# ViacheslavTimofeev/tpu_superresolution

Hardware: AMD Instinct MI355X
Metric: HR pixels/sec, SwinIR x4 train step, 64x64 LR, bs=32/GPU (higher is better)
Workload: dtype bf16; 1 GPU; BASELINE cfg3: SwinIR classical x4 (dim 180, 6x6 blocks, window 8) train step = fwd + L1 + bwd + clip 1.0 + AdamW, 64x64 LR patches -> 256x256 HR, random-init weights, drop_path 0.1; every step starts from the seeded weights and fresh AdamW state; batch_per_gpu=32, global_batch=32, parallelism=dp1

## Files before the change

### tpu_superresolution_amd/csrc/api.hip

```cpp
#include <stdarg.h>
#include <stdio.h>
#include <string.h>

#include "adamw.h"
#include "kernels.h"
#include "wgrad.h"

static thread_local char g_err[512] = "";

SrkOptTls& srk_opt_tls() {
  static thread_local SrkOptTls t = {};
  return t;
}

static SrkOpt** opt_table() {
  static SrkOpt* table[SRK_NUM_OPTS] = {};
  return table;
}

void srk_opt_register(SrkOpt* o) {
  if (o->id >= 0 && o->id < SRK_NUM_OPTS) opt_table()[o->id] = o;
}

void srk_opt_scope_begin(SrkOptTls* saved) {
// ... 308 lines not shown
  srk_gemm_stream_tune_get(&v[0], &v[1], &v[2], &v[3]);
  return v[which];
}
int tune_set(int which, int value) {
  int v[4];
  srk_gemm_stream_tune_get(&v[0], &v[1], &v[2], &v[3]);
  v[which] = value;
  srk_gemm_stream_tune(v[0], v[1], v[2], v[3]);
  return SRK_OK;
}
int wtune_get(int which) {
  int rows, nt;
  srk_wgrad_stream_tune_get(&rows, &nt);
  return which == 0 ? rows : nt;
}

struct OptEntry {
  const char* name;
  int (*get)();
  int (*set)(int);
};

const OptEntry kOptions[] = {
    {"gemm_stream", [] { return srk_gemm_stream_enabled(); }, [](int v) { srk_gemm_stream_enable(v); return (int)SRK_OK; }},
    {"attn_bwd_fused", [] { return srk_attn_bwd_fused_enabled(); }, [](int v) { srk_attn_bwd_fused_enable(v); return (int)SRK_OK; }},
    {"attn_fused", [] { return srk_attn_fused_mode(); }, [](int v) { srk_attn_fused_enable(v); return (int)SRK_OK; }},
    {"wgrad_stream_w8", [] { return srk_wgrad_w8_enabled(); }, [](int v) { srk_wgrad_w8_enable(v); return (int)SRK_OK; }},
    {"block_light", [] { return srk_block_light_enabled(); }, [](int v) { srk_block_light_enable(v); return (int)SRK_OK; }},
    {"mlp_bwd_fused", [] { return srk_mlp_bwd_fused_enabled(); }, [](int v) { srk_mlp_bwd_fused_enable(v); return (int)SRK_OK; }},
    {"mlp_dgelu_store", [] { return srk_mlp_dgelu_store_enabled(); }, [](int v) { srk_mlp_dgelu_store_enable(v); return (int)SRK_OK; }},
    {"mlp_fused", [] { return srk_mlp_fused_enabled(); }, [](int v) { srk_mlp_fused_enable(v); return (int)SRK_OK; }},
    {"wgrad_stream", [] { return srk_wgrad_stream_enabled(); }, [](int v) { srk_wgrad_stream_enable(v); return (int)SRK_OK; }},
    {"conv_wgrad_taps", [] { return srk_conv_wgrad_taps_mode(); }, [](int v) { srk_conv_wgrad_taps_enable(v); return (int)SRK_OK; }},
    {"wgrad_partials", [] { return srk_wgrad_partials_enabled(); }, [](int v) { srk_wgrad_partials_enable(v); return (int)SRK_OK; }},
    {"wgrad_stream_rows", [] { return wtune_get(0); },
     [](int v) {
       SRK_REQUIRE(v == 32 || v == 64, SRK_E_SHAPE, "wgrad_stream_rows: 32/64");
       srk_wgrad_stream_tune(v, -1);
       return (int)SRK_OK;
     }},
    {"wgrad_stream_nt", [] { return wtune_get(1); }, [](int v) { srk_wgrad_stream_tune(0, v != 0); return (int)SRK_OK; }},
    {"gemm_stream_bm", [] { return tune_get(0); },
     [](int v) {
       SRK_REQUIRE(v == 0 || v == 16 || v == 32 || v == 64, SRK_E_SHAPE, "gemm_stream_bm: 0/16/32/64");
       return tune_set(0, v);
     }},
    {"gemm_stream_ks2", [] { return tune_get(1); }, [](int v) { return tune_set(1, v < 0 ? -1 : (v != 0)); }},
    {"gemm_stream_split", [] { return tune_get(2); }, [](int v) { return tune_set(2, v < 0 ? -1 : (v != 0)); }},
    {"gemm_stream_nb", [] { return tune_get(3); },
     [](int v) {
       SRK_REQUIRE(v == 0 || v == 4 || v == 8, SRK_E_SHAPE, "gemm_stream_nb: 0/4/8");
       return tune_set(3, v);
     }},
    {"probe_stride", [] { return g_probe.stride; },
     [](int v) {
       SRK_REQUIRE(v >= 1 && v <= 1024, SRK_E_SHAPE, "probe_stride: 1..1024");
       g_probe.stride = v;
       return (int)SRK_OK;
     }},
};

const OptEntry* find_option(const char* name) {
  for (const OptEntry& e : kOptions)
    if (strcmp(name, e.name) == 0) return &e;
  return nullptr;
}
// ... 158 lines not shown
```

### tpu_superresolution_amd/csrc/common.h

```cpp
#pragma once
#include <hip/hip_runtime.h>
#include <stdint.h>

#include "../../include/srk.h"

typedef unsigned short bf16_t;
typedef __attribute__((ext_vector_type(8))) short bf16x8_t;
typedef __attribute__((ext_vector_type(4))) short bf16x4_t;
typedef __attribute__((ext_vector_type(4))) float f32x4_t;

#define SRK_WAVE 64

void srk_set_error(const char* fmt, ...);
int srk_check_launch(const char* what);

constexpr int SRK_MAX_DEVICES = 64;
int srk_current_device();
int srk_device_cus();
enum SrkOptId {
  OPT_MLP_FUSED, OPT_MLP_BWD_FUSED, OPT_GEMM_STREAM, OPT_TUNE_BM, OPT_TUNE_KS2, OPT_TUNE_SPLIT, OPT_TUNE_NB, OPT_ATTN_BWD_FUSED,
  OPT_ATTN_FUSED, OPT_BLOCK_LIGHT, OPT_TAPS_ENABLED, OPT_TAPS_DMA, OPT_WGRAD_STREAM, OPT_WGRAD_ROWS, OPT_WGRAD_NT, OPT_WGRAD_W8,
  OPT_WGRAD_PARTIALS, OPT_MLP_DGELU_STORE, SRK_NUM_OPTS
};
struct SrkOptTls {
  int v[SRK_NUM_OPTS];
  unsigned on;
};
SrkOptTls& srk_opt_tls();
struct SrkOpt;
void srk_opt_register(SrkOpt* o);
void srk_opt_scope_begin(SrkOptTls* saved);
void srk_opt_scope_end(const SrkOptTls& saved);
struct SrkOpt {
  int id;
  int value;
  SrkOpt(int id_, int v) : id(id_), value(v) { srk_opt_register(this); }
  operator int() const {
    const SrkOptTls& t = srk_opt_tls();
    return ((t.on >> id) & 1u) ? t.v[id] : value;
  }
  SrkOpt& operator=(int v) {
    SrkOptTls& t = srk_opt_tls();
    if ((t.on >> id) & 1u) t.v[id] = v;
    else value = v;
    return *this;
  }
  SrkOpt(const SrkOpt&) = delete;
  SrkOpt& operator=(const SrkOpt&) = delete;
};

template <class T>
struct SrkPerDevice {
  T v[SRK_MAX_DEVICES] = {};
  T& here() { return v[srk_current_device()]; }
};
// ... 214 lines not shown
```

### tpu_superresolution_amd/csrc/convwgrad.hip

```cpp
#include "wgrad.h"

#ifndef SRK_NT_TAPS
#define SRK_NT_TAPS 0
#endif

namespace {

constexpr int CT = 64;
constexpr int SP = 64 + 16;
constexpr int HALO = CT + 2;
constexpr int XROWS = 3 * HALO;
constexpr int YPIECES = CT * 8 / 256;
constexpr int XPIECES = (XROWS * 8 + 255) / 256;

template <bool SHUF>
__global__ __launch_bounds__(256) void conv_wgrad_taps_kernel(const WgradParams p, int ntiles, int chunks_per) {
  extern __shared__ __attribute__((aligned(16))) unsigned char smem[];
  bf16_t* Ys = reinterpret_cast<bf16_t*>(smem);
  bf16_t* Xs = Ys + 2 * CT * SP;

  const int tid = threadIdx.x, lane = tid & 63;
  const int wave = __builtin_amdgcn_readfirstlane(tid >> 6);
  const int r16 = lane & 15, g = lane >> 4;
  const int logical = xcd_remap(blockIdx.x, gridDim.x);
  const int bsplit = logical / ntiles, btile = logical - bsplit * ntiles;
  const int ntn = p.N / 64;
  const int tn = btile % ntn, tk = btile / ntn;
  const int n0 = tn * 64, k0 = tk * 64;
  const int c_begin = bsplit * chunks_per;
  const int c_end = min(p.M / CT, c_begin + chunks_per);
  if (c_begin >= c_end) return;
  const int hw = p.H * p.W;
// ... 120 lines not shown
      srk_set_error("conv wgrad: cannot reserve %zu bytes of LDS", lds);
      return SRK_E_LAUNCH;
    }
    configured = true;
  }
  const int tiles = (p.N / 64) * (p.K / 64);
  const int nchunks = p.M / CT;
  int splits = 256 / tiles;
  if (splits < 1) splits = 1;
  if (splits > nchunks) splits = nchunks;
  const int chunks_per = cdiv(nchunks, splits);
  splits = cdiv(nchunks, chunks_per);
  srk_probe_pre(FAM_WGRAD_CONV, stream, p.flops, p.bytes);
  hipLaunchKernelGGL((conv_wgrad_taps_kernel<SHUF>), dim3(tiles * splits), dim3(256), lds, stream, p, tiles, chunks_per);
  srk_probe_post(FAM_WGRAD_CONV, stream);
  return srk_check_launch("conv wgrad (all taps)");
}

__device__ uint4 g_zero_page[8];

constexpr int TD_YROWS = CT, TD_STAGE_ROWS = CT + XROWS;
constexpr int TD_STAGE_BYTES = TD_STAGE_ROWS * 128;
constexpr int TD_RING = 4;
constexpr int TD_PIECES = TD_STAGE_ROWS * 8;
constexpr int TD_PPW = TD_PIECES / 4;
constexpr int TD_NI = (TD_PPW + 63) / 64;

__device__ __forceinline__ const bf16_t* tr_addr_swz64(const bf16_t* tile, int rbase, int c0, int lane) {
  const int ll = lane & 15;
  const int row = rbase + (ll >> 2);
  return tile + row * 64 + (((c0 >> 4) ^ ((row >> 1) & 3)) << 4) + ((ll & 3) << 2);
}

template <bool SHUF>
__global__ __launch_bounds__(256) void conv_wgrad_taps_dma_kernel(const WgradParams p, int ntiles, int chunks_per, float* partial,
                                                                  int nsplit) {
  extern __shared__ __attribute__((aligned(16))) unsigned char smem[];
  const unsigned ring_base = (unsigned)(size_t)smem;
  const int tid = threadIdx.x, lane = tid & 63;
  const int wave = __builtin_amdgcn_readfirstlane(tid >> 6);
  const int r16 = lane & 15, g = lane >> 4;
  const int logical = xcd_remap(blockIdx.x, gridDim.x);
  const int bsplit = logical / ntiles, btile = logical - bsplit * ntiles;
  const int ntn = p.N / 64;
  const int tn = btile % ntn, tk = btile / ntn;
  const int n0 = tn * 64, k0 = tk * 64;
  const int c_begin = bsplit * chunks_per;
  const int c_end = min(p.M / CT, c_begin + chunks_per);
  if (c_begin >= c_end) return;
  const int hw = p.H * p.W;
  const bf16_t* zero = reinterpret_cast<const bf16_t*>(g_zero_page);

  int loff[TD_NI];
  int lrp[TD_NI];
#pragma unroll
  for (int i = 0; i < TD_NI; ++i) {
    const int qq = wave * TD_PPW + i * 64 + lane;
    const int row = qq >> 3, pos = qq & 7;
    const int c = (((pos >> 1) ^ ((row >> 1) & 3)) << 1) | (pos & 1);
    if (row < TD_YROWS) {
      lrp[i] = -1;
      if constexpr (SHUF) {
        const int nn = n0 + c * 8;
        const int ij = nn / p.Cs, cc = nn - ij * p.Cs;
        const int si = ij / p.r, sj = ij - si * p.r;
        loff[i] = (si * (p.W * p.r) + row * p.r + sj) * p.Cs + cc;
      } else {
        loff[i] = row * p.ldy + n0 + c * 8;
      }
    } else {
// ... 42 lines not shown
    if (it + TD_RING - 2 < nrun) srk_wait_vmcnt<TD_NI*(TD_RING - 2)>(); else srk_wait_vmcnt<0>();
    srk_lds_barrier();
    if (it + TD_RING - 1 < nrun) issue(c_begin + it + TD_RING - 1);
    const bf16_t* ys = reinterpret_cast<const bf16_t*>(smem + (it % TD_RING) * TD_STAGE_BYTES);
    const bf16_t* xs = ys + TD_YROWS * 64;
#pragma unroll
    for (int ks = 0; ks < 2; ++ks) {
      bf16x8_t yf[4];
#pragma unroll
      for (int i = 0; i < 4; ++i) {
        const bf16x4_t lo = lds_tr_read(tr_addr_swz64(ys, 32 * ks + 4 * g, 16 * i, lane));
        const bf16x4_t hi = lds_tr_read(tr_addr_swz64(ys, 32 * ks + 16 + 4 * g, 16 * i, lane));
        yf[i] = bf16x8_t{lo[0], lo[1], lo[2], lo[3], hi[0], hi[1], hi[2], hi[3]};
      }
#pragma unroll
      for (int q = 0; q < 9; ++q) {
        const int cg = 9 * wave + q;
        const int tap = cg >> 2;
        const int xb = (tap / 3) * HALO + (tap % 3);
        const bf16x4_t lo = lds_tr_read(tr_addr_swz64(ys, TD_YROWS + xb + 32 * ks + 4 * g, 16 * (cg & 3), lane));
        const bf16x4_t hi = lds_tr_read(tr_addr_swz64(ys, TD_YROWS + xb + 32 * ks + 16 + 4 * g, 16 * (cg & 3), lane));
        const bf16x8_t xf = bf16x8_t{lo[0], lo[1], lo[2], lo[3], hi[0], hi[1], hi[2], hi[3]};
#pragma unroll
        for (int i = 0; i < 4; ++i) acc[i][q] = __builtin_amdgcn_mfma_f32_16x16x32_bf16(yf[i], xf, acc[i][q], 0, 0, 0);
      }
      if (do_bias) {
#pragma unroll
        for (int i = 0; i < 4; ++i) accb[i] = __builtin_amdgcn_mfma_f32_16x16x32_bf16(yf[i], ones, accb[i], 0, 0, 0);
      }
    }
    (void)xs;
  }

  if (partial != nullptr) {
    f32x4_t* slab = reinterpret_cast<f32x4_t*>(partial) + ((size_t)btile * nsplit + bsplit) * WS_SLAB_VEC + (size_t)wave * 36 * 64 + lane;
#pragma unroll
    for (int i = 0; i < 4; ++i)
#pragma unroll
      for (int q = 0; q < 9; ++q) slab[(i * 9 + q) * 64] = acc[i][q];
  }
#pragma unroll
  for (int i = 0; i < 4; ++i) {
    const int n = n0 + 16 * i + 4 * g;
    if (partial == nullptr) {
#pragma unroll
      for (int q = 0; q < 9; ++q) {
        const int cg = 9 * wave + q;
        const long long col = (long long)(cg >> 2) * p.K + k0 + 16 * (cg & 3) + r16;
#pragma unroll
        for (int e = 0; e < 4; ++e) atomicAdd(p.dW + (long long)(n + e) * p.ldw + col, acc[i][q][e]);
      }
    }
    if (do_bias && r16 == 0) {
#pragma unroll
      for (int e = 0; e < 4; ++e) atomicAdd(p.db + n + e, accb[i][e]);
    }
  }
}

__global__ __launch_bounds__(256) void conv_wgrad_taps_reduce_kernel(const WgradParams p, const float* __restrict__ partial, int nsplit) {
  const int btile = blockIdx.x / 36;
  const int v = (blockIdx.x - btile * 36) * 256 + threadIdx.x;
  const int ntn = p.N / 64;
  const int tn = btile % ntn, tk = btile / ntn;
  const f32x4_t* src = reinterpret_cast<const f32x4_t*>(partial) + (size_t)btile * nsplit * WS_SLAB_VEC + v;
  f32x4_t sum = f32x4_t{0.f, 0.f, 0.f, 0.f};
  int s = 0;
  for (; s + 8 <= nsplit; s += 8) {
    f32x4_t t[8];
#pragma unroll
    for (int u = 0; u < 8; ++u) t[u] = src[(size_t)(s + u) * WS_SLAB_VEC];
#pragma unroll
    for (int u = 0; u < 8; ++u) sum += t[u];
  }
  for (; s < nsplit; ++s) sum += src[(size_t)s * WS_SLAB_VEC];
  const int lane = v & 63, t = v >> 6;
  const int q = t % 9, i = (t / 9) % 4, wave = t / 36;
  const int r16 = lane & 15, g = lane >> 4;
  const int n = tn * 64 + 16 * i + 4 * g;
  const int cg = 9 * wave + q;
  const long long col = (long long)(cg >> 2) * p.K + tk * 64 + 16 * (cg & 3) + r16;
#pragma unroll
  for (int e = 0; e < 4; ++e) atomicAdd(p.dW + (long long)(n + e) * p.ldw + col, sum[e]);
}

SrkOpt g_taps_dma{OPT_TAPS_DMA, 1};

template <bool SHUF>
int launch_taps_dma(const WgradParams& p, hipStream_t stream) {
  constexpr int lds = TD_RING * TD_STAGE_BYTES;
  static SrkPerDevice<bool> configured_pd; bool& configured = configured_pd.here();
  if (!configured) {
    if (hipFuncSetAttribute(reinterpret_cast<const void*>(&conv_wgrad_taps_dma_kernel<SHUF>), hipFuncAttributeMaxDynamicSharedMemorySize,
                            lds) != hipSuccess) {
      srk_set_error("conv wgrad (dma): cannot reserve %d bytes of LDS", lds);
      return SRK_E_LAUNCH;
    }
    configured = true;
  }
  const int tiles = (p.N / 64) * (p.K / 64);
  const int nchunks = p.M / CT;
  int splits = 256 / tiles;
  if (splits < 1) splits = 1;
  if (splits > nchunks) splits = nchunks;
  const int chunks_per = cdiv(nchunks, splits);
  splits = cdiv(nchunks, chunks_per);
  float* partial =
      srk_wgrad_partials_enabled() && splits > 1 ? srk_wgrad_scratch(stream, (size_t)tiles * splits * WS_SLAB_VEC * 16) : nullptr;
  srk_probe_pre(FAM_WGRAD_CONV, stream, p.flops, p.bytes);
  hipLaunchKernelGGL((conv_wgrad_taps_dma_kernel<SHUF>), dim3(tiles * splits), dim3(256), lds, stream, p, tiles, chunks_per, partial,
                     splits);
  if (partial) hipLaunchKernelGGL(conv_wgrad_taps_reduce_kernel, dim3(tiles * 36), dim3(256), 0, stream, p, partial, splits);
  srk_probe_post(FAM_WGRAD_CONV, stream);
  return srk_check_launch("conv wgrad (all taps, dma)");
}

template <int COP>
__global__ __launch_bounds__(256) void smallconv_wgrad_mfma_kernel(const bf16_t* __restrict__ x, const float* __restrict__ gy,
                                                                   float* __restrict__ dW, float* __restrict__ db, int B, int H, int W,
                                                                   int Cin, int CinP, int Co, int ntiles, int chunks_per) {
  extern __shared__ __attribute__((aligned(16))) unsigned char smem[];
  bf16_t* Yh = reinterpret_cast<bf16_t*>(smem);
  bf16_t* Yl = Yh + 2 * CT * 16;
  bf16_t* Xs = Yl + 2 * CT * 16;
  const int tid = threadIdx.x, lane = tid & 63;
  const int wave = __builtin_amdgcn_readfirstlane(tid >> 6);
  const int r16 = lane & 15, g = lane >> 4;
  const int logical = xcd_remap(blockIdx.x, gridDim.x);
  const int bsplit = logical / ntiles, tk = logical - bsplit * ntiles;
  const int k0 = tk * 64;
  const int M = B * H * W;
  const int c_begin = bsplit * chunks_per;
  const int c_end = min(M / CT, c_begin + chunks_per);
  if (c_begin >= c_end) return;
  const int hw = H * W;
  for (int i = tid; i < 2 * 2 * CT * 16 / 2; i += 256) reinterpret_cast<unsigned*>(Yh)[i] = 0u;

  constexpr int YP = CT * COP / 4;
  float4 ry = make_float4(0.f, 0.f, 0.f, 0.f);
  uint4 rx[XPIECES];
  const int nxb = W / CT;
  auto load_stage = [&](int ch) {
    const int b = ch / (H * nxb), r = ch - b * (H * nxb);
    const int xb = r / H, y = r - xb * H, x0 = xb * CT;
    const int m0 = b * hw + y * W + x0;
    if (tid < YP) ry = *reinterpret_cast<const float4*>(gy + (long long)m0 * COP + tid * 4);
#pragma unroll
    for (int t = 0; t < XPIECES; ++t) {
      const int pid = tid + 256 * t;
      const int hr = pid >> 3, c8 = pid & 7;
      const int rr = hr / HALO, px = hr - rr * HALO;
// ... 62 lines not shown
        const bf16x8_t xf = bf16x8_t{lo[0], lo[1], lo[2], lo[3], hi[0], hi[1], hi[2], hi[3]};
        acc[q] = __builtin_amdgcn_mfma_f32_16x16x32_bf16(yfh, xf, acc[q], 0, 0, 0);
        acc[q] = __builtin_amdgcn_mfma_f32_16x16x32_bf16(yfl, xf, acc[q], 0, 0, 0);
      }
      if (do_bias) {
        accb = __builtin_amdgcn_mfma_f32_16x16x32_bf16(yfh, ones, accb, 0, 0, 0);
        accb = __builtin_amdgcn_mfma_f32_16x16x32_bf16(yfl, ones, accb, 0, 0, 0);
      }
    }
    if (ch + 1 < c_end) store_stage(buf ^ 1);
    __syncthreads();
  }

#pragma unroll
  for (int q = 0; q < 9; ++q) {
    const int cg = 9 * wave + q;
    const int tap = cg >> 2, k = k0 + 16 * (cg & 3) + r16;
#pragma unroll
    for (int e = 0; e < 4; ++e) {
      const int n = 4 * g + e;
      if (n < Co && k < Cin) atomicAdd(dW + ((long long)(n * Cin) + k) * 9 + tap, acc[q][e]);
    }
  }
  if (do_bias && r16 == 0) {
#pragma unroll
    for (int e = 0; e < 4; ++e)
      if (4 * g + e < Co) atomicAdd(db + 4 * g + e, accb[e]);
  }
}

template <int COP>
int launch_smallconv_mfma(const bf16_t* x, const float* gy, float* dW, float* db, int B, int H, int W, int Cin, int CinP, int Co,
                          hipStream_t stream) {
  constexpr size_t lds = (size_t)(2 * 2 * CT * 16 + 2 * XROWS * SP) * sizeof(bf16_t);
  static SrkPerDevice<bool> configured_pd; bool& configured = configured_pd.here();
  if (!configured) {
    if (hipFuncSetAttribute(reinterpret_cast<const void*>(&smallconv_wgrad_mfma_kernel<COP>), hipFuncAttributeMaxDynamicSharedMemorySize,
                            (int)lds) != hipSuccess) {
      srk_set_error("smallconv wgrad: cannot reserve %zu bytes of LDS", lds);
      return SRK_E_LAUNCH;
    }
    configured = true;
  }
  const int tiles = CinP / 64;
  const int nchunks = (B * H * W) / CT;
  int splits = 512 / tiles;
  if (splits > nchunks) splits = nchunks;
  const int chunks_per = cdiv(nchunks, splits);
  splits = cdiv(nchunks, chunks_per);
  hipLaunchKernelGGL((smallconv_wgrad_mfma_kernel<COP>), dim3(tiles * splits), dim3(256), lds, stream, x, gy, dW, db, B, H, W, Cin, CinP, Co,
                     tiles, chunks_per);
  return srk_check_launch("smallconv wgrad (mfma)");
}

__device__ __forceinline__ void split_bf16x8(const float (&v)[8], bf16x8_t& hi, bf16x8_t& lo) {
#pragma unroll
  for (int i = 0; i < 8; ++i) {
    const bf16_t h = f2bf(v[i]);
    hi[i] = (short)h;
    lo[i] = (short)f2bf(v[i] - bf2f(h));
  }
}

__global__ __launch_bounds__(256) void imghead_dgrad_mfma_kernel(const float* __restrict__ gy, const float* __restrict__ wgt,
                                                                 bf16_t* __restrict__ dx, int B, int H, int W, int Cin, int Co, int nchunks) {
  constexpr int TP = 64 + 8;
  __shared__ __attribute__((aligned(16))) bf16_t T[64 * TP];
  const int tid = threadIdx.x, lane = tid & 63;
  const int wave = __builtin_amdgcn_readfirstlane(tid >> 6);
  const int r16 = lane & 15, g = lane >> 4;

  bf16x8_t wh[4][2], wl[4][2];
#pragma unroll
  for (int j = 0; j < 4; ++j)
#pragma unroll
    for (int ks = 0; ks < 2; ++ks) {
      float v[8];
#pragma unroll
      for (int jj = 0; jj < 8; ++jj) {
        const int k = 32 * ks + 8 * g + jj;
        const int tap = k >> 2, co = k & 3, ci = 16 * j + r16;
        v[jj] = (tap < 9 && co < Co && ci < Cin) ? wgt[((co * Cin) + ci) * 9 + tap] : 0.f;
      }
      split_bf16x8(v, wh[j][ks], wl[j][ks]);
    }

  const int hw = H * W;
  for (int c = blockIdx.x; c < nchunks; c += gridDim.x) {
    const int pix = c * 64 + 16 * wave + r16;
    const int b = pix / hw, rem = pix - b * hw;
    const int y = rem / W, x = rem - y * W;
    f32x4_t acc[4];
#pragma unroll
    for (int j = 0; j < 4; ++j) acc[j] = f32x4_t{0.f, 0.f, 0.f, 0.f};
// ... 11 lines not shown
        }
        v[4 * half] = gv.x; v[4 * half + 1] = gv.y; v[4 * half + 2] = gv.z; v[4 * half + 3] = gv.w;
      }
      bf16x8_t xh, xl;
      split_bf16x8(v, xh, xl);
#pragma unroll
      for (int j = 0; j < 4; ++j) {
        acc[j] = __builtin_amdgcn_mfma_f32_16x16x32_bf16(wh[j][ks], xh, acc[j], 0, 0, 0);
        acc[j] = __builtin_amdgcn_mfma_f32_16x16x32_bf16(wl[j][ks], xh, acc[j], 0, 0, 0);
        acc[j] = __builtin_amdgcn_mfma_f32_16x16x32_bf16(wh[j][ks], xl, acc[j], 0, 0, 0);
      }
    }
#pragma unroll
    for (int j = 0; j < 4; ++j)
      *reinterpret_cast<uint2*>(T + (16 * wave + r16) * TP + 16 * j + 4 * g) = pack_bf4(acc[j][0], acc[j][1], acc[j][2], acc[j][3]);
    srk_lds_barrier();
#pragma unroll
    for (int t = 0; t < 2; ++t) {
      const int pid = tid + 256 * t;
      const int row = pid >> 3, c8 = pid & 7;
      *reinterpret_cast<uint4*>(dx + ((long long)c * 64 + row) * 64 + c8 * 8) = *reinterpret_cast<const uint4*>(T + row * TP + c8 * 8);
    }
    srk_lds_barrier();
  }
}

}

void srk_conv_wgrad_taps_enable(int on) {
  g_taps_enabled = on ? 1 : 0;
  g_taps_dma = on >= 2 ? 1 : 0;
}
int srk_conv_wgrad_taps_mode() { return g_taps_enabled ? (g_taps_dma ? 2 : 1) : 0; }

int srk_launch_conv_wgrad_taps(const WgradParams& p, hipStream_t stream) {
  if (!g_taps_enabled || !p.conv || p.W % CT != 0 || p.N % 64 != 0 || p.K % 64 != 0 || p.ldx % 8 != 0) return SRK_WGRAD_NOT_COVERED;
  if (p.r > 1) {
    if (p.Cs % 8 != 0 || p.N != p.r * p.r * p.Cs) return SRK_WGRAD_NOT_COVERED;
    return g_taps_dma ? launch_taps_dma<true>(p, stream) : launch_taps<true>(p, stream);
  }
  if (p.ldy % 8 != 0) return SRK_WGRAD_NOT_COVERED;
  return g_taps_dma ? launch_taps_dma<false>(p, stream) : launch_taps<false>(p, stream);
}

int srk_launch_smallconv_wgrad_mfma(const bf16_t* x, const float* gy, float* dW, float* db, int B, int H, int W, int Cin, int CinP,
                                    int Co, int CoP, hipStream_t stream) {
  if (!g_taps_enabled || W % CT != 0 || CinP % 64 != 0 || Co > CoP || ((long long)B * H * W) % CT != 0) return SRK_WGRAD_NOT_COVERED;
  if (CoP == 4) return launch_smallconv_mfma<4>(x, gy, dW, db, B, H, W, Cin, CinP, Co, stream);
  if (CoP == 16) return launch_smallconv_mfma<16>(x, gy, dW, db, B, H, W, Cin, CinP, Co, stream);
  return SRK_WGRAD_NOT_COVERED;
}

int srk_launch_imghead_dgrad_mfma(const float* gy, const float* wgt, bf16_t* dx, int B, int H, int W, int Cin, int CinP, int Co, int CoP,
                                  hipStream_t stream) {
  const long long npix = (long long)B * H * W;
  if (!g_taps_enabled || CoP != 4 || CinP != 64 || Co > 4 || Cin > 64 || npix % 64 != 0 || npix > (1ll << 30)) return SRK_WGRAD_NOT_COVERED;
  const int nchunks = (int)(npix / 64);
  const int grid = nchunks < 2048 ? nchunks : 2048;
  hipLaunchKernelGGL(imghead_dgrad_mfma_kernel, dim3(grid), dim3(256), 0, stream, gy, wgt, dx, B, H, W, Cin, Co, nchunks);
  return srk_check_launch("image-head dgrad (mfma)");
}
```

### tpu_superresolution_amd/csrc/wgrad.h

```cpp
#pragma once
#include "common.h"

struct WgradParams {
  const bf16_t* Y;
  int ldy;
  const bf16_t* X;
  int ldx;
  int M, N, K;
  float* dW;
  int ldw;
  float* db;
  int m_per;
  int conv;
  int B, H, W;
  double flops;
  double bytes;
  int r, Cs;
};

struct RpbJob {
  const float* slab;
  float* dtable;
  int nslab, nH;
};
// ... 18 lines not shown
  int sidx = wave;
  for (; sidx + 28 < nslab; sidx += 32) {
#pragma unroll
    for (int u = 0; u < 8; ++u) a8[u] += base[(sidx + 4 * u) * sstride];
  }
  for (; sidx < nslab; sidx += 4) a8[0] += base[sidx * sstride];
  part[wave][lane] = ((a8[0] + a8[1]) + (a8[2] + a8[3])) + ((a8[4] + a8[5]) + (a8[6] + a8[7]));
  __syncthreads();
  if (wave == 0) {
    const float v = part[0][lane] + part[1][lane] + part[2][lane] + part[3][lane];
    const int t = ((i >> 3) - (lane >> 3) + 7) * 15 + ((i & 7) - (lane & 7) + 7);
    atomicAdd(dtable + t * nH + h, v);
  }
}

constexpr int WS_SLAB_VEC = 9216;
constexpr size_t WS_WORKSPACE_BYTES = (size_t)256 * WS_SLAB_VEC * 16;
float* srk_wgrad_scratch(hipStream_t stream, size_t bytes);
void srk_wgrad_bind_workspace(void* ptr, size_t bytes, void** prev_ptr, size_t* prev_bytes);
void srk_wgrad_partials_enable(int on);
void srk_wgrad_w8_enable(int on);
void srk_wgrad_stream_tune(int rows, int nt);
int srk_wgrad_partials_enabled();
int srk_wgrad_stream_enabled();
int srk_wgrad_w8_enabled();
void srk_wgrad_stream_tune_get(int* rows, int* nt);

int srk_launch_wgrad(const WgradParams& p, hipStream_t stream);

#define SRK_WGRAD_NOT_COVERED 1
int srk_launch_conv_wgrad_taps(const WgradParams& p, hipStream_t stream);
void srk_conv_wgrad_taps_enable(int on);
int srk_conv_wgrad_taps_mode();
int srk_launch_smallconv_wgrad_mfma(const bf16_t* x, const float* gy, float* dW, float* db, int B, int H, int W, int Cin, int CinP, int Co,
                                    int CoP, hipStream_t stream);
int srk_launch_imghead_dgrad_mfma(const float* gy, const float* wgt, bf16_t* dx, int B, int H, int W, int Cin, int CinP, int Co, int CoP,
                                  hipStream_t stream);
void srk_wgrad_stream_enable(int on);
int srk_launch_wgrad_multi(const WgradParams* ps, int nprob, hipStream_t stream);
int srk_launch_wgrad_multi_rpb(const WgradParams* ps, int nprob, const RpbJob* rpb, hipStream_t stream);
int srk_launch_rpb_reduce(const float* slab, float* dtable, int nslab, int nH, hipStream_t stream);
```

Baseline: 74.97 million HR pixels/s.

## Add rolling-row LDS window for conv weight-gradient kernels

Adds a rolling row-buffer variant of the 3x3 conv weight-gradient DMA kernel and the small-conv MFMA kernel. Input rows are kept in an LDS ring and reused across the three vertical taps, instead of restaging a halo of three rows for every chunk. Work is now split per image row (one or two 64-pixel chunks per row), and LDS is sized so two workgroups fit per CU. Both paths are on by default behind a new option. The cost is more complex indexing and stricter shape conditions (W of 64 or 128), with the old staged kernels kept as fallback.

```diff
diff --git a/tpu_superresolution_amd/csrc/api.hip b/tpu_superresolution_amd/csrc/api.hip
--- a/tpu_superresolution_amd/csrc/api.hip
+++ b/tpu_superresolution_amd/csrc/api.hip
@@ -364,6 +364,7 @@
     {"mlp_fused", [] { return srk_mlp_fused_enabled(); }, [](int v) { srk_mlp_fused_enable(v); return (int)SRK_OK; }},
     {"wgrad_stream", [] { return srk_wgrad_stream_enabled(); }, [](int v) { srk_wgrad_stream_enable(v); return (int)SRK_OK; }},
     {"conv_wgrad_taps", [] { return srk_conv_wgrad_taps_mode(); }, [](int v) { srk_conv_wgrad_taps_enable(v); return (int)SRK_OK; }},
+    {"conv_wgrad_roll", [] { return srk_conv_wgrad_roll_enabled(); }, [](int v) { srk_conv_wgrad_roll_enable(v); return (int)SRK_OK; }},
     {"wgrad_partials", [] { return srk_wgrad_partials_enabled(); }, [](int v) { srk_wgrad_partials_enable(v); return (int)SRK_OK; }},
     {"wgrad_stream_rows", [] { return wtune_get(0); },
      [](int v) {
diff --git a/tpu_superresolution_amd/csrc/common.h b/tpu_superresolution_amd/csrc/common.h
--- a/tpu_superresolution_amd/csrc/common.h
+++ b/tpu_superresolution_amd/csrc/common.h
@@ -20,7 +20,7 @@
 enum SrkOptId {
   OPT_MLP_FUSED, OPT_MLP_BWD_FUSED, OPT_GEMM_STREAM, OPT_TUNE_BM, OPT_TUNE_KS2, OPT_TUNE_SPLIT, OPT_TUNE_NB, OPT_ATTN_BWD_FUSED,
   OPT_ATTN_FUSED, OPT_BLOCK_LIGHT, OPT_TAPS_ENABLED, OPT_TAPS_DMA, OPT_WGRAD_STREAM, OPT_WGRAD_ROWS, OPT_WGRAD_NT, OPT_WGRAD_W8,
-  OPT_WGRAD_PARTIALS, OPT_MLP_DGELU_STORE, SRK_NUM_OPTS
+  OPT_WGRAD_PARTIALS, OPT_MLP_DGELU_STORE, OPT_TAPS_ROLL, SRK_NUM_OPTS
 };
 struct SrkOptTls {
   int v[SRK_NUM_OPTS];
diff --git a/tpu_superresolution_amd/csrc/convwgrad.hip b/tpu_superresolution_amd/csrc/convwgrad.hip
--- a/tpu_superresolution_amd/csrc/convwgrad.hip
+++ b/tpu_superresolution_amd/csrc/convwgrad.hip
@@ -1,3 +1,5 @@
+#include <type_traits>
+
 #include "wgrad.h"
 
 #ifndef SRK_NT_TAPS
@@ -184,10 +186,38 @@
   return tile + row * 64 + (((c0 >> 4) ^ ((row >> 1) & 3)) << 4) + ((ll & 3) << 2);
 }
 
+__device__ __forceinline__ void taps_store(const WgradParams& p, const f32x4_t (&acc)[4][9], const f32x4_t (&accb)[4], float* partial,
+                                           int nsplit, int btile, int bsplit, int wave, int lane, int n0, int k0, bool do_bias) {
+  const int r16 = lane & 15, g = lane >> 4;
+  if (partial != nullptr) {
+    f32x4_t* slab = reinterpret_cast<f32x4_t*>(partial) + ((size_t)btile * nsplit + bsplit) * WS_SLAB_VEC + (size_t)wave * 36 * 64 + lane;
+#pragma unroll
+    for (int i = 0; i < 4; ++i)
+#pragma unroll
+      for (int q = 0; q < 9; ++q) slab[(i * 9 + q) * 64] = acc[i][q];
+  }
+#pragma unroll
+  for (int i = 0; i < 4; ++i) {
+    const int n = n0 + 16 * i + 4 * g;
+    if (partial == nullptr) {
+#pragma unroll
+      for (int q = 0; q < 9; ++q) {
+        const int cg = 9 * wave + q;
+        const long long col = (long long)(cg >> 2) * p.K + k0 + 16 * (cg & 3) + r16;
+#pragma unroll
+        for (int e = 0; e < 4; ++e) atomicAdd(p.dW + (long long)(n + e) * p.ldw + col, acc[i][q][e]);
+      }
+    }
+    if (do_bias && r16 == 0) {
+#pragma unroll
+      for (int e = 0; e < 4; ++e) atomicAdd(p.db + n + e, accb[i][e]);
+    }
+  }
+}
+
 template <bool SHUF>
-__global__ __launch_bounds__(256) void conv_wgrad_taps_dma_kernel(const WgradParams p, int ntiles, int chunks_per, float* partial,
-                                                                  int nsplit) {
-  extern __shared__ __attribute__((aligned(16))) unsigned char smem[];
+__device__ __forceinline__ void taps_dma_staged(const WgradParams& p, int ntiles, int chunks_per, float* partial, int nsplit,
+                                                unsigned char* smem) {
   const unsigned ring_base = (unsigned)(size_t)smem;
   const int tid = threadIdx.x, lane = tid & 63;
   const int wave = __builtin_amdgcn_readfirstlane(tid >> 6);
@@ -296,30 +326,218 @@
     (void)xs;
   }
 
-  if (partial != nullptr) {
-    f32x4_t* slab = reinterpret_cast<f32x4_t*>(partial) + ((size_t)btile * nsplit + bsplit) * WS_SLAB_VEC + (size_t)wave * 36 * 64 + lane;
-#pragma unroll
-    for (int i = 0; i < 4; ++i)
-#pragma unroll
-      for (int q = 0; q < 9; ++q) slab[(i * 9 + q) * 64] = acc[i][q];
-  }
+  taps_store(p, acc, accb, partial, nsplit, btile, bsplit, wave, lane, n0, k0, do_bias);
+}
+
+template <int RPR>
+struct RL {
+  static constexpr int A = RPR == 1 ? 4 : 3;
+  static constexpr int PRO = 3 * RPR - 1;
+  static constexpr int NY = A + 1;
+  static constexpr int NR = (A + PRO + RPR - 1) / RPR + 1;
+  static constexpr int ROWB = (RPR * CT + 2) * 128;
+  static constexpr int X_OFF = NY * CT * 128, Z_OFF = X_OFF + NR * ROWB, LDS = Z_OFF + HALO * 128;
+};
+
+template <bool NT = false>
+__device__ __forceinline__ void srk_glds16_s2(const void* sb0, const void* sb1, unsigned voff, unsigned dst0, unsigned dst1) {
+  unsigned keep;
+  if constexpr (NT)
+    asm volatile("s_mov_b32 %0, m0\n\ts_mov_b32 m0, %2\n\ts_nop 0\n\tglobal_load_lds_dwordx4 %1, %4 nt\n\ts_mov_b32 m0, %3\n\ts_nop 0\n\t"
+                 "global_load_lds_dwordx4 %1, %5 nt\n\ts_mov_b32 m0, %0"
+                 : "=&s"(keep)
+                 : "v"(voff), "s"(dst0), "s"(dst1), "s"(sb0), "s"(sb1)
+                 : "memory");
+  else
+    asm volatile("s_mov_b32 %0, m0\n\ts_mov_b32 m0, %2\n\ts_nop 0\n\tglobal_load_lds_dwordx4 %1, %4\n\ts_mov_b32 m0, %3\n\ts_nop 0\n\t"
+                 "global_load_lds_dwordx4 %1, %5\n\ts_mov_b32 m0, %0"
+                 : "=&s"(keep)
+                 : "v"(voff), "s"(dst0), "s"(dst1), "s"(sb0), "s"(sb1)
+                 : "memory");
+}
+
+__device__ __forceinline__ bf16x4_t lds_tr_read_at(unsigned addr) {
+  typedef __attribute__((ext_vector_type(4))) short s4;
+  return __builtin_amdgcn_ds_read_tr16_b64_v4i16((s4 __attribute__((address_space(3)))*)(addr));
+}
+
+template <bool SHUF, int RPR>
+__device__ __forceinline__ void taps_dma_roll(const WgradParams& p, int ntiles, int chunks_per, float* partial, int nsplit,
+                                              unsigned char* smem) {
+  using C = RL<RPR>;
+  const unsigned lds0 = (unsigned)(size_t)smem;
+  const int tid = threadIdx.x, lane = tid & 63;
+  const int wave = __builtin_amdgcn_readfirstlane(tid >> 6);
+  const int logical = xcd_remap(blockIdx.x, gridDim.x);
+  const int bsplit = logical / ntiles, btile = logical - bsplit * ntiles;
+  const int ntn = p.N / 64;
+  const int tn = btile % ntn, tk = btile / ntn;
+  const int n0 = tn * 64, k0 = tk * 64;
+  const int c_begin = bsplit * chunks_per;
+  const int c_end = min(p.M / CT, c_begin + chunks_per);
+  if (c_begin >= c_end) return;
+  const int nrun = c_end - c_begin;
+  const int BH = p.B * p.H;
+  const int G0 = c_begin / RPR;
+  int y = G0 % p.H;
+
+  for (int i = tid; i < HALO * 8; i += 256) *reinterpret_cast<uint4*>(smem + C::Z_OFF + i * 16) = make_uint4(0, 0, 0, 0);
+  for (int i = tid; i < C::NR * 16; i += 256)
+    *reinterpret_cast<uint4*>(smem + C::X_OFF + (i >> 4) * C::ROWB + ((i >> 3) & 1) * (RPR * CT + 1) * 128 + (i & 7) * 16) =
+        make_uint4(0, 0, 0, 0);
+
+  const int l8 = lane >> 3, pos = lane & 7;
+  const int cy = (((pos >> 1) ^ ((l8 >> 1) & 3)) << 1) | (pos & 1);
+  const int cx = (((pos >> 1) ^ (((l8 + 1) >> 1) & 3)) << 1) | (pos & 1);
+  unsigned voffy;
+  int ypix;
+  if constexpr (SHUF) {
+    const int nn = n0 + cy * 8;
+    const int ij = nn / p.Cs, cc = nn - ij * p.Cs;
+    const int si = ij / p.r, sj = ij - si * p.r;
+    voffy = 2u * (unsigned)((si * (p.W * p.r) + l8 * p.r + sj) * p.Cs + cc);
+    ypix = p.r * p.Cs;
+  } else {
+    voffy = 2u * (unsigned)(l8 * p.ldy + n0 + cy * 8);
+    ypix = p.ldy;
+  }
+  const unsigned voffx = 2u * (unsigned)(l8 * p.ldx + k0 + cx * 8);
+
+  const long long y8 = (long long)8 * ypix * 2, x8 = (long long)8 * p.ldx * 2;
+  const long long ystep_in = (long long)CT * ypix * 2;
+  const long long ystep_row = SHUF ? ((long long)p.r * (p.W * p.r) - (long long)(RPR - 1) * CT * p.r) * p.Cs * 2 : ystep_in;
+  const long long xstep_in = (long long)CT * p.ldx * 2, xstep_row = (long long)p.W * p.ldx * 2;
+  const unsigned ydst0 = lds0 + (unsigned)(wave * 2048), ydst_end = ydst0 + C::NY * (CT * 128);
+  const unsigned xdst0 = lds0 + (unsigned)(C::X_OFF + (1 + wave * 16) * 128), xdst_end = xdst0 + C::NR * C::ROWB;
+  const char* ysrc = reinterpret_cast<const char*>(
+      p.Y + (SHUF ? (long long)G0 * p.r * (p.W * p.r) * p.Cs : (long long)c_begin * CT * p.ldy) + (long long)(wave * 16) * ypix);
+  int xj = G0 - 1;
+  const char* xsrc = reinterpret_cast<const char*>(p.X + ((long long)max(xj, 0) * p.W + wave * 16) * p.ldx);
+  unsigned ydst = ydst0, xdst = xdst0;
+  int yh = 0, xh = 0;
+  auto issue_y = [&]() {
+    srk_glds16_s2<SRK_NT_TAPS != 0>(ysrc, ysrc + y8, voffy, ydst, ydst + 1024);
+    ydst = ydst + CT * 128 == ydst_end ? ydst0 : ydst + CT * 128;
+    if (RPR == 1 || ++yh == RPR) {
+      yh = 0;
+      ysrc += ystep_row;
+    } else {
+      ysrc += ystep_in;
+    }
+  };
+  auto issue_x = [&]() {
+    const char* s = RPR == 1 ? xsrc : xsrc + xh * xstep_in;
+    const unsigned d = RPR == 1 ? xdst : xdst + (unsigned)(xh * (CT * 128));
+    srk_glds16_s2<SRK_NT_TAPS != 0>(s, s + x8, voffx, d, d + 1024);
+    if (RPR == 1 || ++xh == RPR) {
+      xh = 0;
+      xdst = xdst + C::ROWB == xdst_end ? xdst0 : xdst + C::ROWB;
+      ++xj;
+      if (xj > 0 && xj < BH) xsrc += xstep_row;
+    }
+  };
+
+  const int g = lane >> 4, ll = lane & 15;
+  const int lrow = 4 * g + (ll >> 2);
+  unsigned yoff[4], xoff[9];
+#pragma unroll
+  for (int i = 0; i < 4; ++i) yoff[i] = (unsigned)(lrow * 128 + ((i ^ ((lrow >> 1) & 3)) << 5) + ((ll & 3) << 3));
+  const int dA = ((9 * wave) >> 2) / 3, dB = ((9 * wave + 8) >> 2) / 3;
+  int nsel = 0;
+#pragma unroll
+  for (int q = 0; q < 9; ++q) {
+    const int cg = 9 * wave + q;
+    const int tap = cg >> 2, kf = cg & 3;
+    const int px = tap % 3 + lrow;
+    nsel += tap / 3 == dA ? 1 : 0;
+    xoff[q] = (unsigned)(px * 128 + ((kf ^ ((px >> 1) & 3)) << 5) + ((ll & 3) << 3));
+  }
+
+  f32x4_t acc[4][9], accb[4];
 #pragma unroll
   for (int i = 0; i < 4; ++i) {
-    const int n = n0 + 16 * i + 4 * g;
-    if (partial == nullptr) {
+    accb[i] = f32x4_t{0.f, 0.f, 0.f, 0.f};
+#pragma unroll
+    for (int q = 0; q < 9; ++q) acc[i][q] = f32x4_t{0.f, 0.f, 0.f, 0.f};
+  }
+  const bool do_bias = p.db != nullptr && tk == 0 && wave == 0;
+  const bf16x8_t ones = bf16x8_t{0x3F80, 0x3F80, 0x3F80, 0x3F80, 0x3F80, 0x3F80, 0x3F80, 0x3F80};
+
+  for (int uu = 0; uu < C::PRO; ++uu) issue_x();
+  for (int k = 0; k < C::A && k < nrun; ++k) {
+    issue_y();
+    issue_x();
+  }
+  const unsigned xbeg = lds0 + C::X_OFF, xend = xbeg + C::NR * C::ROWB, zrow = lds0 + C::Z_OFF;
+  unsigned ys = lds0, xs0 = xbeg, xs1 = xbeg + C::ROWB, xs2 = xbeg + 2 * C::ROWB;
+  int u = 0;
+  auto run_loop = [&](auto bias) {
+  constexpr bool BIAS = decltype(bias)::value;
+  for (int it = 0; it < nrun; ++it) {
+    if (it + C::A - 1 < nrun) srk_wait_vmcnt<4 * (C::A - 1)>(); else srk_wait_vmcnt<0>();
+    srk_lds_barrier();
+    if (it + C::A < nrun) {
+      issue_y();
+      issue_x();
+    }
+    const unsigned xu = (unsigned)(u * (CT * 128));
+    const unsigned rb0 = y > 0 ? xs0 + xu : zrow;
+    const unsigned rb1 = xs1 + xu;
+    const unsigned rb2 = y + 1 < p.H ? xs2 + xu : zrow;
+    const unsigned rbA = dA == 0 ? rb0 : (dA == 1 ? rb1 : rb2);
+    const unsigned rbB = dB == 0 ? rb0 : (dB == 1 ? rb1 : rb2);
+#pragma unroll
+    for (int ks = 0; ks < 2; ++ks) {
+      bf16x8_t yf[4];
+#pragma unroll
+      for (int i = 0; i < 4; ++i) {
+        const bf16x4_t lo = lds_tr_read_at(ys + yoff[i] + (32 * ks) * 128);
+        const bf16x4_t hi = lds_tr_read_at(ys + yoff[i] + (32 * ks + 16) * 128);
+        yf[i] = bf16x8_t{lo[0], lo[1], lo[2], lo[3], hi[0], hi[1], hi[2], hi[3]};
+      }
 #pragma unroll
       for (int q = 0; q < 9; ++q) {
-        const int cg = 9 * wave + q;
-        const long long col = (long long)(cg >> 2) * p.K + k0 + 16 * (cg & 3) + r16;
-#pragma unroll
-        for (int e = 0; e < 4; ++e) atomicAdd(p.dW + (long long)(n + e) * p.ldw + col, acc[i][q][e]);
-      }
-    }
-    if (do_bias && r16 == 0) {
-#pragma unroll
-      for (int e = 0; e < 4; ++e) atomicAdd(p.db + n + e, accb[i][e]);
-    }
-  }
+        const unsigned rb = q < nsel ? rbA : rbB;
+        const bf16x4_t lo = lds_tr_read_at(rb + xoff[q] + (32 * ks) * 128);
+        const bf16x4_t hi = lds_tr_read_at(rb + xoff[q] + (32 * ks + 16) * 128);
+        const bf16x8_t xf = bf16x8_t{lo[0], lo[1], lo[2], lo[3], hi[0], hi[1], hi[2], hi[3]};
+#pragma unroll
+        for (int i = 0; i < 4; ++i) acc[i][q] = __builtin_amdgcn_mfma_f32_16x16x32_bf16(yf[i], xf, acc[i][q], 0, 0, 0);
+      }
+      if constexpr (BIAS) {
+#pragma unroll
+        for (int i = 0; i < 4; ++i) accb[i] = __builtin_amdgcn_mfma_f32_16x16x32_bf16(yf[i], ones, accb[i], 0, 0, 0);
+      }
+    }
+    ys = ys + CT * 128 == xbeg ? lds0 : ys + CT * 128;
+    if (RPR == 1 || ++u == RPR) {
+      u = 0;
+      xs0 = xs1;
+      xs1 = xs2;
+      xs2 = xs2 + C::ROWB == xend ? xbeg : xs2 + C::ROWB;
+      y = y + 1 == p.H ? 0 : y + 1;
+    }
+  }
+  };
+  if (do_bias) run_loop(std::true_type{});
+  else run_loop(std::false_type{});
+
+  taps_store(p, acc, accb, partial, nsplit, btile, bsplit, wave, lane, n0, k0, do_bias);
+}
+
+template <bool SHUF>
+__global__ __launch_bounds__(256, 2) void conv_wgrad_taps_dma_kernel(const WgradParams p, int ntiles, int chunks_per, float* partial,
+                                                                     int nsplit, int rpr) {
+  extern __shared__ __attribute__((aligned(16))) unsigned char smem[];
+  if (rpr == 1) taps_dma_roll<SHUF, 1>(p, ntiles, chunks_per, partial, nsplit, smem);
+  else taps_dma_roll<SHUF, 2>(p, ntiles, chunks_per, partial, nsplit, smem);
+}
+
+template <bool SHUF>
+__global__ __launch_bounds__(256) void conv_wgrad_taps_dma_staged_kernel(const WgradParams p, int ntiles, int chunks_per, float* partial,
+                                                                         int nsplit) {
+  extern __shared__ __attribute__((aligned(16))) unsigned char smem[];
+  taps_dma_staged<SHUF>(p, ntiles, chunks_per, partial, nsplit, smem);
 }
 
 __global__ __launch_bounds__(256) void conv_wgrad_taps_reduce_kernel(const WgradParams p, const float* __restrict__ partial, int nsplit) {
@@ -349,21 +567,29 @@
 }
 
 SrkOpt g_taps_dma{OPT_TAPS_DMA, 1};
+SrkOpt g_taps_roll{OPT_TAPS_ROLL, 1};
 
 template <bool SHUF>
 int launch_taps_dma(const WgradParams& p, hipStream_t stream) {
-  constexpr int lds = TD_RING * TD_STAGE_BYTES;
+  constexpr int lds_staged = TD_RING * TD_STAGE_BYTES;
+  constexpr int lds_roll = RL<2>::LDS > RL<1>::LDS ? RL<2>::LDS : RL<1>::LDS;
+  static_assert(lds_roll <= 160 * 1024 && lds_staged <= 160 * 1024, "LDS budget");
   static SrkPerDevice<bool> configured_pd; bool& configured = configured_pd.here();
   if (!configured) {
     if (hipFuncSetAttribute(reinterpret_cast<const void*>(&conv_wgrad_taps_dma_kernel<SHUF>), hipFuncAttributeMaxDynamicSharedMemorySize,
-                            lds) != hipSuccess) {
-      srk_set_error("conv wgrad (dma): cannot reserve %d bytes of LDS", lds);
+                            lds_roll) != hipSuccess ||
+        hipFuncSetAttribute(reinterpret_cast<const void*>(&conv_wgrad_taps_dma_staged_kernel<SHUF>),
+                            hipFuncAttributeMaxDynamicSharedMemorySize, lds_staged) != hipSuccess) {
+      srk_set_error("conv wgrad (dma): cannot reserve %d bytes of LDS", lds_roll > lds_staged ? lds_roll : lds_staged);
       return SRK_E_LAUNCH;
     }
     configured = true;
   }
+  const int rpr = g_taps_roll && (p.W == CT || p.W == 2 * CT) && p.M % p.W == 0 ? p.W / CT : 0;
+  const int lds = rpr == 1 ? RL<1>::LDS : (rpr == 2 ? RL<2>::LDS : lds_staged);
+  const int unit = rpr ? rpr : 1;
   const int tiles = (p.N / 64) * (p.K / 64);
-  const int nchunks = p.M / CT;
+  const int nchunks = p.M / CT / unit;
   int splits = 256 / tiles;
   if (splits < 1) splits = 1;
   if (splits > nchunks) splits = nchunks;
@@ -372,15 +598,216 @@
   float* partial =
       srk_wgrad_partials_enabled() && splits > 1 ? srk_wgrad_scratch(stream, (size_t)tiles * splits * WS_SLAB_VEC * 16) : nullptr;
   srk_probe_pre(FAM_WGRAD_CONV, stream, p.flops, p.bytes);
-  hipLaunchKernelGGL((conv_wgrad_taps_dma_kernel<SHUF>), dim3(tiles * splits), dim3(256), lds, stream, p, tiles, chunks_per, partial,
-                     splits);
+  if (rpr)
+    hipLaunchKernelGGL((conv_wgrad_taps_dma_kernel<SHUF>), dim3(tiles * splits), dim3(256), lds, stream, p, tiles, chunks_per * unit,
+                       partial, splits, rpr);
+  else
+    hipLaunchKernelGGL((conv_wgrad_taps_dma_staged_kernel<SHUF>), dim3(tiles * splits), dim3(256), lds, stream, p, tiles, chunks_per,
+                       partial, splits);
   if (partial) hipLaunchKernelGGL(conv_wgrad_taps_reduce_kernel, dim3(tiles * 36), dim3(256), 0, stream, p, partial, splits);
   srk_probe_post(FAM_WGRAD_CONV, stream);
   return srk_check_launch("conv wgrad (all taps, dma)");
 }
 
+__device__ __forceinline__ void split_bf16x8(const float (&v)[8], bf16x8_t& hi, bf16x8_t& lo) {
+#pragma unroll
+  for (int i = 0; i < 8; ++i) {
+    const bf16_t h = f2bf(v[i]);
+    hi[i] = (short)h;
+    lo[i] = (short)f2bf(v[i] - bf2f(h));
+  }
+}
+
 template <int COP>
-__global__ __launch_bounds__(256) void smallconv_wgrad_mfma_kernel(const bf16_t* __restrict__ x, const float* __restrict__ gy,
+struct SR {
+  static constexpr int A = 3, NY = A + 1, NR = A + 3;
+  static constexpr int GYB = CT * COP * 4;
+  static constexpr int ROWB = HALO * 128;
+  static constexpr int X_OFF = NY * GYB, Z_OFF = X_OFF + NR * ROWB, LDS = Z_OFF + ROWB;
+};
+
+template <bool NT = false>
+__device__ __forceinline__ void srk_glds16_s1(const void* sb, unsigned voff, unsigned dst) {
+  unsigned keep;
+  asm volatile("s_mov_b32 %0, m0\n\ts_mov_b32 m0, %2\n\ts_nop 0\n\tglobal_load_lds_dwordx4 %1, %3\n\ts_mov_b32 m0, %0"
+               : "=&s"(keep)
+               : "v"(voff), "s"(dst), "s"(sb)
+               : "memory");
+}
+
+__device__ __forceinline__ float lds_read_f32(unsigned addr) {
+  return *reinterpret_cast<const float __attribute__((address_space(3)))*>(addr);
+}
+
+template <int COP>
+__global__ __launch_bounds__(256, 2) void smallconv_wgrad_mfma_kernel(const bf16_t* __restrict__ x, const float* __restrict__ gy,
+                                                                      float* __restrict__ dW, float* __restrict__ db, int B, int H, int W,
+                                                                      int Cin, int CinP, int Co, int ntiles, int chunks_per) {
+  using C = SR<COP>;
+  extern __shared__ __attribute__((aligned(16))) unsigned char smem[];
+  const unsigned lds0 = (unsigned)(size_t)smem;
+  const int tid = threadIdx.x, lane = tid & 63;
+  const int wave = __builtin_amdgcn_readfirstlane(tid >> 6);
+  const int logical = xcd_remap(blockIdx.x, gridDim.x);
+  const int bsplit = logical / ntiles, tk = logical - bsplit * ntiles;
+  const int k0 = tk * 64;
+  const int NCH = (int)(((long long)B * H * W) / CT);
+  const int c_begin = bsplit * chunks_per;
+  const int c_end = min(NCH, c_begin + chunks_per);
+  if (c_begin >= c_end) return;
+  const int nrun = c_end - c_begin;
+  const int nxb = W / CT;
+  for (int i = tid; i < HALO * 8; i += 256) *reinterpret_cast<uint4*>(smem + C::Z_OFF + i * 16) = make_uint4(0, 0, 0, 0);
+
+  auto locate = [&](int ch, int& cy, int& cxb) -> long long {
+    const int b = ch / (H * nxb), r = ch - b * (H * nxb);
+    cxb = r / H;
+    cy = r - cxb * H;
+    return ((long long)(b * H + cy)) * W + cxb * CT;
+  };
+  auto step = [&](int& cy, int& cxb, const char*& ptr, long long ebytes) {
+    if (++cy == H) {
+      cy = 0;
+      if (++cxb == nxb) {
+        cxb = 0;
+        ptr += CT * ebytes;
+      } else {
+        ptr += ((long long)CT - (long long)(H - 1) * W) * ebytes;
+      }
+    } else {
+      ptr += (long long)W * ebytes;
+    }
+  };
+  const long long xe = (long long)CinP * 2, ge = (long long)COP * 4;
+  int xj = c_begin - 1, xy, xxb, gyy, gxb, y;
+  const char* xptr = reinterpret_cast<const char*>(x + k0) + locate(max(xj, 0), xy, xxb) * xe;
+  const char* gptr = reinterpret_cast<const char*>(gy) + locate(c_begin, gyy, gxb) * ge;
+  y = gyy;
+  const char* zero = reinterpret_cast<const char*>(g_zero_page);
+
+  constexpr int LA = CT * COP / 16;
+  const int l8 = lane >> 3, pos = lane & 7;
+  const unsigned voffx = 2u * (unsigned)(l8 * CinP + ((((pos >> 1) ^ ((l8 >> 1) & 3)) << 1) | (pos & 1)) * 8);
+  const unsigned voffh = (unsigned)(((wave & 1) * 4 + (lane & 3)) * 16);
+  const unsigned voffg = (unsigned)((lane & (LA - 1)) * 16);
+  const unsigned gdst0 = lds0 + (unsigned)(wave * LA * 16), gdst_end = gdst0 + C::NY * C::GYB;
+  const unsigned xdst0 = lds0 + C::X_OFF, xdst_end = xdst0 + C::NR * C::ROWB;
+  unsigned gdst = gdst0, xdst = xdst0;
+  auto issue_y = [&]() {
+    if (LA == 64 || lane < LA) srk_glds16_s1(gptr + wave * LA * 16, voffg, gdst);
+    gdst = gdst + C::GYB == gdst_end ? gdst0 : gdst + C::GYB;
+    step(gyy, gxb, gptr, ge);
+  };
+  auto issue_x = [&]() {
+    const char* s = xptr + (long long)(wave * 16) * xe;
+    const unsigned d = xdst + (unsigned)(wave * 2048);
+    srk_glds16_s2(s, s + 8 * xe, voffx, d, d + 1024);
+    const bool ok = wave < 2 ? xxb + 1 < nxb : xxb > 0;
+    const char* hb = ok ? (wave < 2 ? xptr + CT * xe : xptr - xe) : zero;
+    if (lane < 4) srk_glds16_s1(hb, voffh, xdst + (unsigned)(CT * 128 + wave * 64));
+    xdst = xdst + C::ROWB == xdst_end ? xdst0 : xdst + C::ROWB;
+    ++xj;
+    if (xj > 0 && xj < NCH) step(xy, xxb, xptr, xe);
+  };
+
+  const int g = lane >> 4, ll = lane & 15;
+  const int lrow = 4 * g + (ll >> 2);
+  const unsigned goff = (unsigned)((4 * g) * COP * 4 + (ll < COP ? ll : 0) * 4);
+  unsigned xoff0[9];
+  int xoff[9];
+  const int dA = ((9 * wave) >> 2) / 3, dB = ((9 * wave + 8) >> 2) / 3;
+  int nsel = 0;
+#pragma unroll
+  for (int q = 0; q < 9; ++q) {
+    const int cg = 9 * wave + q;
+    const int tap = cg >> 2, kf = cg & 3;
+    const int pr = lrow + tap % 3 - 1;
+    const int p0 = pr < 0 ? HALO - 1 : pr, p1 = pr + 16;
+    nsel += tap / 3 == dA ? 1 : 0;
+    xoff0[q] = (unsigned)(p0 * 128 + ((kf ^ ((p0 >> 1) & 3)) << 5) + ((ll & 3) << 3));
+    xoff[q] = p1 * 128 + ((kf ^ ((p1 >> 1) & 3)) << 5) + ((ll & 3) << 3) - 16 * 128;
+  }
+
+  f32x4_t acc[9], accb = f32x4_t{0.f, 0.f, 0.f, 0.f};
+#pragma unroll
+  for (int q = 0; q < 9; ++q) acc[q] = f32x4_t{0.f, 0.f, 0.f, 0.f};
+  const bool do_bias = db != nullptr && tk == 0 && wave == 0;
+  const bf16x8_t ones = bf16x8_t{0x3F80, 0x3F80, 0x3F80, 0x3F80, 0x3F80, 0x3F80, 0x3F80, 0x3F80};
+
+  issue_x();
+  issue_x();
+  for (int k = 0; k < C::A && k < nrun; ++k) {
+    issue_y();
+    issue_x();
+  }
+  const unsigned zrow = lds0 + C::Z_OFF;
+  unsigned gs = lds0, xs0 = xdst0, xs1 = xdst0 + C::ROWB, xs2 = xdst0 + 2 * C::ROWB;
+  auto run_loop = [&](auto bias) {
+  constexpr bool BIAS = decltype(bias)::value;
+  for (int it = 0; it < nrun; ++it) {
+    if (it + C::A - 1 < nrun) srk_wait_vmcnt<4 * (C::A - 1)>(); else srk_wait_vmcnt<0>();
+    srk_lds_barrier();
+    if (it + C::A < nrun) {
+      issue_y();
+      issue_x();
+    }
+    const unsigned rb0 = y > 0 ? xs0 : zrow;
+    const unsigned rb2 = y + 1 < H ? xs2 : zrow;
+    const unsigned rbA = dA == 0 ? rb0 : (dA == 1 ? xs1 : rb2);
+    const unsigned rbB = dB == 0 ? rb0 : (dB == 1 ? xs1 : rb2);
+#pragma unroll
+    for (int ks = 0; ks < 2; ++ks) {
+      float v[8];
+#pragma unroll
+      for (int jj = 0; jj < 8; ++jj) {
+        const float t = lds_read_f32(gs + goff + (unsigned)((32 * ks + 16 * (jj >> 2) + (jj & 3)) * COP * 4));
+        v[jj] = ll < COP ? t : 0.f;
+      }
+      bf16x8_t yfh, yfl;
+      split_bf16x8(v, yfh, yfl);
+#pragma unroll
+      for (int q = 0; q < 9; ++q) {
+        const unsigned rb = q < nsel ? rbA : rbB;
+        const bf16x4_t lo = lds_tr_read_at(ks == 0 ? rb + xoff0[q] : rb + (unsigned)xoff[q] + 32 * 128);
+        const bf16x4_t hi = lds_tr_read_at(rb + (unsigned)xoff[q] + (32 * ks + 16) * 128);
+        const bf16x8_t xf = bf16x8_t{lo[0], lo[1], lo[2], lo[3], hi[0], hi[1], hi[2], hi[3]};
+        acc[q] = __builtin_amdgcn_mfma_f32_16x16x32_bf16(yfh, xf, acc[q], 0, 0, 0);
+        acc[q] = __builtin_amdgcn_mfma_f32_16x16x32_bf16(yfl, xf, acc[q], 0, 0, 0);
+      }
+      if constexpr (BIAS) {
+        accb = __builtin_amdgcn_mfma_f32_16x16x32_bf16(yfh, ones, accb, 0, 0, 0);
+        accb = __builtin_amdgcn_mfma_f32_16x16x32_bf16(yfl, ones, accb, 0, 0, 0);
+      }
+    }
+    gs = gs + C::GYB == lds0 + C::X_OFF ? lds0 : gs + C::GYB;
+    xs0 = xs1;
+    xs1 = xs2;
+    xs2 = xs2 + C::ROWB == xdst_end ? xdst0 : xs2 + C::ROWB;
+    y = y + 1 == H ? 0 : y + 1;
+  }
+  };
+  if (do_bias) run_loop(std::true_type{});
+  else run_loop(std::false_type{});
+
+#pragma unroll
+  for (int q = 0; q < 9; ++q) {
+    const int cg = 9 * wave + q;
+    const int tap = cg >> 2, k = k0 + 16 * (cg & 3) + ll;
+#pragma unroll
+    for (int e = 0; e < 4; ++e) {
+      const int n = 4 * g + e;
+      if (n < Co && k < Cin) atomicAdd(dW + ((long long)(n * Cin) + k) * 9 + tap, acc[q][e]);
+    }
+  }
+  if (do_bias && ll == 0) {
+#pragma unroll
+    for (int e = 0; e < 4; ++e)
+      if (4 * g + e < Co) atomicAdd(db + 4 * g + e, accb[e]);
+  }
+}
+
+template <int COP>
+__global__ __launch_bounds__(256) void smallconv_wgrad_mfma_staged_kernel(const bf16_t* __restrict__ x, const float* __restrict__ gy,
                                                                    float* __restrict__ dW, float* __restrict__ db, int B, int H, int W,
                                                                    int Cin, int CinP, int Co, int ntiles, int chunks_per) {
   extern __shared__ __attribute__((aligned(16))) unsigned char smem[];
@@ -509,34 +936,32 @@
 template <int COP>
 int launch_smallconv_mfma(const bf16_t* x, const float* gy, float* dW, float* db, int B, int H, int W, int Cin, int CinP, int Co,
                           hipStream_t stream) {
-  constexpr size_t lds = (size_t)(2 * 2 * CT * 16 + 2 * XROWS * SP) * sizeof(bf16_t);
+  constexpr int lds_staged = (int)((2 * 2 * CT * 16 + 2 * XROWS * SP) * sizeof(bf16_t));
+  static_assert(2 * SR<COP>::LDS <= 160 * 1024, "two workgroups per CU");
   static SrkPerDevice<bool> configured_pd; bool& configured = configured_pd.here();
   if (!configured) {
     if (hipFuncSetAttribute(reinterpret_cast<const void*>(&smallconv_wgrad_mfma_kernel<COP>), hipFuncAttributeMaxDynamicSharedMemorySize,
-                            (int)lds) != hipSuccess) {
-      srk_set_error("smallconv wgrad: cannot reserve %zu bytes of LDS", lds);
+                            SR<COP>::LDS) != hipSuccess ||
+        hipFuncSetAttribute(reinterpret_cast<const void*>(&smallconv_wgrad_mfma_staged_kernel<COP>),
+                            hipFuncAttributeMaxDynamicSharedMemorySize, lds_staged) != hipSuccess) {
+      srk_set_error("smallconv wgrad: cannot reserve %d bytes of LDS", SR<COP>::LDS > lds_staged ? SR<COP>::LDS : lds_staged);
       return SRK_E_LAUNCH;
     }
     configured = true;
   }
   const int tiles = CinP / 64;
-  const int nchunks = (B * H * W) / CT;
+  const int nchunks = (int)(((long long)B * H * W) / CT);
   int splits = 512 / tiles;
   if (splits > nchunks) splits = nchunks;
   const int chunks_per = cdiv(nchunks, splits);
   splits = cdiv(nchunks, chunks_per);
-  hipLaunchKernelGGL((smallconv_wgrad_mfma_kernel<COP>), dim3(tiles * splits), dim3(256), lds, stream, x, gy, dW, db, B, H, W, Cin, CinP, Co,
-                     tiles, chunks_per);
+  if (g_taps_roll)
+    hipLaunchKernelGGL((smallconv_wgrad_mfma_kernel<COP>), dim3(tiles * splits), dim3(256), SR<COP>::LDS, stream, x, gy, dW, db, B, H, W,
+                       Cin, CinP, Co, tiles, chunks_per);
+  else
+    hipLaunchKernelGGL((smallconv_wgrad_mfma_staged_kernel<COP>), dim3(tiles * splits), dim3(256), lds_staged, stream, x, gy, dW, db, B, H,
+                       W, Cin, CinP, Co, tiles, chunks_per);
   return srk_check_launch("smallconv wgrad (mfma)");
-}
-
-__device__ __forceinline__ void split_bf16x8(const float (&v)[8], bf16x8_t& hi, bf16x8_t& lo) {
-#pragma unroll
-  for (int i = 0; i < 8; ++i) {
-    const bf16_t h = f2bf(v[i]);
-    hi[i] = (short)h;
-    lo[i] = (short)f2bf(v[i] - bf2f(h));
-  }
 }
 
 __global__ __launch_bounds__(256) void imghead_dgrad_mfma_kernel(const float* __restrict__ gy, const float* __restrict__ wgt,
@@ -614,6 +1039,8 @@
   g_taps_dma = on >= 2 ? 1 : 0;
 }
 int srk_conv_wgrad_taps_mode() { return g_taps_enabled ? (g_taps_dma ? 2 : 1) : 0; }
+void srk_conv_wgrad_roll_enable(int on) { g_taps_roll = on ? 1 : 0; }
+int srk_conv_wgrad_roll_enabled() { return g_taps_roll; }
 
 int srk_launch_conv_wgrad_taps(const WgradParams& p, hipStream_t stream) {
   if (!g_taps_enabled || !p.conv || p.W % CT != 0 || p.N % 64 != 0 || p.K % 64 != 0 || p.ldx % 8 != 0) return SRK_WGRAD_NOT_COVERED;
diff --git a/tpu_superresolution_amd/csrc/wgrad.h b/tpu_superresolution_amd/csrc/wgrad.h
--- a/tpu_superresolution_amd/csrc/wgrad.h
+++ b/tpu_superresolution_amd/csrc/wgrad.h
@@ -74,6 +74,8 @@
 int srk_launch_conv_wgrad_taps(const WgradParams& p, hipStream_t stream);
 void srk_conv_wgrad_taps_enable(int on);
 int srk_conv_wgrad_taps_mode();
+void srk_conv_wgrad_roll_enable(int on);
+int srk_conv_wgrad_roll_enabled();
 int srk_launch_smallconv_wgrad_mfma(const bf16_t* x, const float* gy, float* dW, float* db, int B, int H, int W, int Cin, int CinP, int Co,
                                     int CoP, hipStream_t stream);
 int srk_launch_imghead_dgrad_mfma(const float* gy, const float* wgt, bf16_t* dx, int B, int H, int W, int Cin, int CinP, int Co, int CoP,
```

Result: faster. 76.28 million HR pixels/s (median of 6 runs) (+1.7%).
